# cule/multimot_track

Measured on AMD Instinct MI355X. Metric: KITTI RGB-D frames/sec (ego+object poses) at 1/2/4/8 GPUs; CPU ref fps, higher is better.
Workload: dtype u8

## Files before the change

multimot_track_amd/csrc/mmt_bowmap.hip:

```cpp

#include <algorithm>
#include <climits>
#include <cmath>
#include <cstring>
#include <functional>

#include "mmt_internal.h"
#include "mmt_map.h"
#include "mmt_mat4.h"
#include "mmt_pnp.h"

namespace mmt {

namespace {
constexpr int TH_LOW = 50, HISTO_LENGTH = 30;

void three_max(const std::vector<int>* histo, int& ind1, int& ind2, int& ind3) {
  int max1 = 0, max2 = 0, max3 = 0;
  for (int i = 0; i < HISTO_LENGTH; i++) {
    const int s = (int)histo[i].size();
    if (s > max1) {
      max3 = max2; max2 = max1; max1 = s;
      ind3 = ind2; ind2 = ind1; ind1 = i;
    } else if (s > max2) {
// ... 816 lines not shown
        const float errX1 = u1 - kp1.x, errY1 = v1 - kp1.y;
        if ((errX1 * errX1 + errY1 * errY1) > 5.991 * sigmaSquare1) continue;
      } else {
        const float u1 = cam_.fx * x1 * invz1 + cam_.cx;
        const float u1_r = u1 - cam_.bf * invz1;
        const float v1 = cam_.fy * y1 * invz1 + cam_.cy;
        const float errX1 = u1 - kp1.x, errY1 = v1 - kp1.y, errX1_r = u1_r - kp1_ur;
        if ((errX1 * errX1 + errY1 * errY1 + errX1_r * errX1_r) > 7.8 * sigmaSquare1) continue;
      }
      const float sc2 = cam_.scale[kp2.octave], sigmaSquare2 = sc2 * sc2;
      const float x2 = row_dot(T2, 0), y2 = row_dot(T2, 1);
      const float invz2 = (float)(1.0 / z2);
      if (!bStereo2) {
        const float u2 = cam_.fx * x2 * invz2 + cam_.cx, v2 = cam_.fy * y2 * invz2 + cam_.cy;
        const float errX2 = u2 - kp2.x, errY2 = v2 - kp2.y;
        if ((errX2 * errX2 + errY2 * errY2) > 5.991 * sigmaSquare2) continue;
      } else {
        const float u2 = cam_.fx * x2 * invz2 + cam_.cx;
        const float u2_r = u2 - cam_.bf * invz2;
        const float v2 = cam_.fy * y2 * invz2 + cam_.cy;
        const float errX2 = u2 - kp2.x, errY2 = v2 - kp2.y, errX2_r = u2_r - kp2_ur;
        if ((errX2 * errX2 + errY2 * errY2 + errX2_r * errX2_r) > 7.8 * sigmaSquare2) continue;
      }
      const float n1v[3] = {x3D[0] - kfs_[kf].Ow[0], x3D[1] - kfs_[kf].Ow[1], x3D[2] - kfs_[kf].Ow[2]};
      const float n2v[3] = {x3D[0] - kfs_[k2].Ow[0], x3D[1] - kfs_[k2].Ow[1], x3D[2] - kfs_[k2].Ow[2]};
      const float dist1 = norm3(n1v), dist2 = norm3(n2v);
      if (dist1 == 0 || dist2 == 0) continue;
      const float ratioDist = dist2 / dist1;
      const float ratioOctave = cam_.scale[kp1.octave] / cam_.scale[kp2.octave];
      if (ratioDist * ratioFactor < ratioOctave || ratioDist > ratioOctave * ratioFactor) continue;
      const int hnew = new_point_kf(x3D, kf);
      add_observation(hnew, kf, idx1);
      add_observation(hnew, k2, idx2);
      kfs_[kf].mps[idx1] = hnew;
      kfs_[k2].mps[idx2] = hnew;
      compute_distinctive(hnew);
      update_normal_depth(hnew);
      recent_.push_back(hnew);
      bstats_.n_triangulated++;
    }
  }
}

}
```

multimot_track_amd/csrc/mmt_localmap.hip:

```cpp

#include <hip/hip_runtime.h>

#include <algorithm>
#include <climits>
#include <cmath>
#include <cstring>
#include <map>
#include <set>

#include "mmt_map.h"
#include "mmt_mat4.h"

namespace mmt {

void MapEngine::grow_dev(uint8_t*& d, uint8_t*& h, size_t& cap, size_t need) {
  if (need <= cap && d) return;
  const size_t c = std::max(need + (need >> 1), (size_t)1 << 16);
  if (d) {
    MMT_HIP(hipStreamSynchronize(lm_s_));
    dallocs_.erase(std::find(dallocs_.begin(), dallocs_.end(), (void*)d));
    (void)hipFree(d);
    hallocs_.erase(std::find(hallocs_.begin(), hallocs_.end(), (void*)h));
    (void)hipHostFree(h);
  }
// ... 32 lines not shown
  memcpy(K.Tcw, T, 64);
  cam_centre(T, K.Ow);
  mat4_eye(K.Twc);
  for (int r = 0; r < 3; r++) {
    for (int c = 0; c < 3; c++) K.Twc[4 * r + c] = T[4 * c + r];
    K.Twc[4 * r + 3] = K.Ow[r];
  }
}

void MapEngine::erase_observation(int h, int kf) {
  MPoint& p = mp(h);
  auto it = std::lower_bound(p.obs.begin(), p.obs.end(), std::make_pair(kf, INT_MIN));
  if (it == p.obs.end() || it->first != kf) return;
  if (kfs_[kf].uR[it->second] >= 0)
    p.nObs -= 2;
  else
    p.nObs--;
  p.obs.erase(it);
  if (p.refKF == kf) p.refKF = p.obs.empty() ? -1 : p.obs.front().first;
  if (p.nObs <= 2) set_bad(h);
}

void MapEngine::replace(int h, int by) {
  if (h == by) return;
  MPoint& p = mp(h);
  const std::vector<std::pair<int, int>> obs = p.obs;
  p.obs.clear();
  mark_bad(h);
  const int nvisible = p.visible, nfound = p.found;
  p.replaced = by;
  mark_dirty(h);
  for (const auto& kv : obs) {
    if (mp(by).obs_index(kv.first) < 0) {
      kfs_[kv.first].mps[kv.second] = by;
      add_observation(by, kv.first, kv.second);
    } else {
      kfs_[kv.first].mps[kv.second] = -1;
    }
  }
  MPoint& q = mp(by);
  q.found += nfound;
  q.visible += nvisible;
  compute_distinctive(by);
}

void MapEngine::erase_connection(int kf, int other) {
  if (kfs_[kf].conn.erase(other)) update_best_covisibles(kf);
}

void MapEngine::kf_set_bad(int kf) {
  KFrame& K = kfs_[kf];
  if (K.id == 0) return;
  for (const auto& kv : std::map<int, int>(K.conn)) erase_connection(kv.first, kf);
  for (size_t i = 0; i < K.mps.size(); i++)
    if (K.mps[i] >= 0) erase_observation(K.mps[i], kf);
  K.conn.clear();
  K.ordered.clear();
  std::set<int> cand;
  cand.insert(K.parent);
  while (!K.children.empty()) {
    bool bContinue = false;
    int mx = -1, pC = -1, pP = -1;
    for (int ch : K.children) {
      if (kfs_[ch].bad) continue;
      for (int c : kfs_[ch].ordered)
        for (int q : cand)
          if (c == q) {
            auto it = kfs_[ch].conn.find(c);
            const int wgt = it == kfs_[ch].conn.end() ? 0 : it->second;
            if (wgt > mx) {
              pC = ch;
              pP = c;
              mx = wgt;
              bContinue = true;
            }
          }
    }
    if (!bContinue) break;
    kfs_[pC].parent = pP;
    kfs_[pP].children.insert(pC);
    mstats_.n_reparent++;
    cand.insert(pC);
    K.children.erase(pC);
  }
  if (K.parent >= 0) {
    for (int ch : K.children) {
      kfs_[ch].parent = K.parent;
      kfs_[K.parent].children.insert(ch);
      mstats_.n_reparent++;
    }
    kfs_[K.parent].children.erase(kf);
  }
  K.bad = true;
  kfdb_erase(kf);
}

void MapEngine::fuse_launch(const std::vector<int>& kft_kf, const std::vector<FuseQuery>& q,
                            int2* res) {
  const int nq = (int)q.size();
  if (nq == 0) return;
  const double t0 = prof_on_ ? now_us() : 0;
  double tq = t0;
  gpu_flush_pool(lm_s_);
  blk_time(10, tq);
  const size_t tb = al16(sizeof(FuseKF) * kft_kf.size());
  grow_dev(d_fup_, h_fup_, fup_cap_, tb + sizeof(FuseQuery) * (size_t)nq);
  {
    uint8_t* dres = (uint8_t*)d_fres_;
    uint8_t* hres = (uint8_t*)h_fres_;
    grow_dev(dres, hres, fres_cap_, sizeof(int2) * (size_t)nq);
    d_fres_ = (int2*)dres;
    h_fres_ = (int2*)hres;
  }
  FuseKF* tab = (FuseKF*)h_fup_;
  for (size_t t = 0; t < kft_kf.size(); t++) {
    const KFrame& K = kfs_[kft_kf[t]];
    tab[t] = K.dev;
    memcpy(tab[t].Tcw, K.Tcw, 64);
    memcpy(tab[t].Ow, K.Ow, 12);
  }
  memcpy(h_fup_ + tb, q.data(), sizeof(FuseQuery) * (size_t)nq);
  MMT_HIP(hipMemcpyAsync(d_fup_, h_fup_, tb + sizeof(FuseQuery) * (size_t)nq,
                         hipMemcpyHostToDevice, lm_s_));
  FuseCam c;
  memset(&c, 0, sizeof(c));
  c.fx = cam_.fx; c.fy = cam_.fy; c.cx = cam_.cx; c.cy = cam_.cy; c.bf = cam_.bf;
// ... 4 lines not shown
  c.logScale = cam_.logScale;
  c.th = 3.f;
  c.nlevels = cam_.nlevels;
  for (int l = 0; l < cam_.nlevels && l < kMaxLevels; l++) {
    c.scale[l] = cam_.scale[l];
    c.invSigma2[l] = cam_.invSigma2[l];
  }
  launch_fuse_cand((const FuseKF*)d_fup_, (const FuseQuery*)(d_fup_ + tb), nq, d_pool_,
                   d_pool_desc_, c, d_fres_, lm_s_);
  MMT_HIP(hipMemcpyAsync(h_fres_, d_fres_, sizeof(int2) * (size_t)nq, hipMemcpyDeviceToHost,
                         lm_s_));
  blk_time(11, tq);
  MMT_HIP(hipStreamSynchronize(lm_s_));
  blk_time(12, tq);
  memcpy(res, h_fres_, sizeof(int2) * (size_t)nq);
  mstats_.fuse_launches++;
  mstats_.fuse_queries += nq;
  if (prof_on_) mstats_.fuse_us += now_us() - t0;
}

void MapEngine::fuse_apply(int kf, int h, int bestIdx, int bestDist) {
  if (bestDist > 50) return;
  KFrame& K = kfs_[kf];
  const int pin = K.mps[bestIdx];
  if (pin >= 0) {
    if (!mp(pin).bad) {
      if (mp(pin).nObs > mp(h).nObs)
        replace(h, pin);
      else
        replace(pin, h);
    }
  } else {
    add_observation(h, kf, bestIdx);
    K.mps[bestIdx] = h;
  }
  mstats_.n_fused++;
}

void MapEngine::fuse_sequence(const std::vector<int>& kfl, const std::vector<int>& pts) {
  const int nk = (int)kfl.size(), np = (int)pts.size();
  if (nk == 0 || np == 0) return;
  std::vector<int> qidx((size_t)nk * np, -1);
  std::vector<FuseQuery> q;
  std::vector<int> ver;
  for (int t = 0; t < nk; t++)
    for (int i = 0; i < np; i++) {
      if (t == 0 && i + 8 < np) prefetch_point(pts[i + 8]);
      const int h = pts[i];
      if (h < 0 || mp(h).bad || mp(h).obs_index(kfl[t]) >= 0) continue;
      qidx[(size_t)t * np + i] = (int)q.size();
      q.push_back(FuseQuery{t, h});
      ver.push_back(mp(h).desc_ver);
    }
  std::vector<int2> res(q.size());
  double tb = prof_on_ ? now_us() : 0;
  fuse_launch(kfl, q, res.data());
  tb = prof_on_ ? now_us() : 0;
  for (int t = 0; t < nk; t++) {
    const int kf = kfl[t];
    for (int i = 0; i < np; i++) {
      const int h = pts[i];
      if (h < 0) continue;
      const MPoint& p = mp(h);
      if (p.bad || p.obs_index(kf) >= 0) continue;
      const int qi = qidx[(size_t)t * np + i];
      if (qi < 0) continue;
      if (ver[qi] != p.desc_ver) {
// ... 135 lines not shown
  for (int v = 0; v < nK; v++) vIdx[verts[v]] = -1;
  BAHostProblem P;
  P.n_kf = nK;
  P.n_pt = nP;
  P.n_edge = nE;
  P.Tcw = Tv.data();
  P.fixed = fixed.data();
  P.Xw = Xv.data();
  P.e_pt = e_pt.data();
  P.e_kf = e_kf.data();
  P.e_obs = e_obs.data();
  P.e_s = e_s.data();
  P.fx = cam_.fx; P.fy = cam_.fy; P.cx = cam_.cx; P.cy = cam_.cy; P.bf = cam_.bf;
  std::vector<float> Tout(16 * (size_t)nK), Xout(3 * (size_t)nP);
  std::vector<uint8_t> er(std::max(nE, 1));
  int st[5];
  double tb = prof_on_ ? now_us() : 0;
  if (prof_on_) mstats_.blk_us[8] += tb - t0;
  ba_.run(P, lm_s_, Tout.data(), Xout.data(), er.data(), st);
  if (prof_on_) mstats_.basolve_us += now_us() - tb;
  tb = prof_on_ ? now_us() : 0;
  mstats_.n_ba++;
  mstats_.ba_trials += st[2] + st[3];
  mstats_.ba_edges += nE;
  mstats_.ba_kfs += nK;
  mstats_.ba_pts += nP;
  mstats_.ba_max_opt = std::max<long>(mstats_.ba_max_opt, nO);
  for (int pass = 0; pass < 2; pass++)
    for (int i = 0; i < nE; i++) {
      const bool stereo = !(e_obs[3 * (size_t)i + 2] < 0);
      if (stereo != (pass == 1) || !er[i]) continue;
      const int h = lpts[e_pt[i]], k = e_kfid[i];
      const int idx = mp(h).obs_index(k);
      if (idx >= 0) kfs_[k].mps[idx] = -1;
      erase_observation(h, k);
      mstats_.n_ba_erased++;
    }
  for (size_t v = 0; v < local.size(); v++) set_pose(local[v], &Tout[16 * v]);
  for (int j = 0; j < nP; j++) {
    MPoint& p = mp(lpts[j]);
    memcpy(p.pos, &Xout[3 * (size_t)j], 12);
    mark_dirty(lpts[j]);
    update_normal_depth(lpts[j]);
  }
  blk_time(9, tb);
  if (prof_on_) mstats_.ba_us += now_us() - t0;
}

void MapEngine::keyframe_culling(int kf) {
  const std::vector<int> local = kfs_[kf].ordered;
  for (int k : local) {
    KFrame& K = kfs_[k];
    if (K.id == 0) continue;
    const int thObs = 3;
    int nRedundant = 0, nMPs = 0;
    for (size_t i = 0; i < K.mps.size(); i++) {
      const int h = K.mps[i];
      if (h < 0) continue;
      const MPoint& p = mp(h);
      if (p.bad) continue;
      if (K.depth[i] > cam_.thDepth || K.depth[i] < 0) continue;
      nMPs++;
      if (p.nObs > thObs) {
        const int scaleLevel = K.keys[i].octave;
        int nObs = 0;
        for (const auto& kv : p.obs) {
          if (kv.first == k) continue;
// ... 38 lines not shown
```

multimot_track_amd/csrc/mmt_map.h:

```cpp
#pragma once
#include <hip/hip_runtime.h>

#include <cstdint>
#include <functional>
#include <map>
#include <set>
#include <unordered_map>
#include <utility>
#include <memory>
#include <vector>

#include "mmt_ba.h"
#include "mmt_bow.h"
#include "mmt_internal.h"
#include "mmt_match.h"
#include "mmt_track.h"

namespace mmt {

struct MapCamH {
  int W = 0, H = 0;
  float fx = 0, fy = 0, cx = 0, cy = 0, invfx = 0, invfy = 0, bf = 0;
  float thDepth = 0;
  int maxFrames = 0;
// ... 150 lines not shown
    const double n = now_us();
    mstats_.blk_us[k] += n - t;
    t = n;
  }
  void prefetch_point(int h) const {
#ifndef MMT_NO_PREFETCH
    if (h >= 0 && h < kTemp && (size_t)h < pts_.size()) __builtin_prefetch(&pts_[h]);
#else
    (void)h;
#endif
  }
  void set_cull_ratio(double r) { cull_ratio_ = r; }
  void dump(int32_t* sizes, const mmt_map_dump_arrays* out) const;
  void set_vocabulary(Vocabulary* v);
  const BowStatsH& bow_stats() const { return bstats_; }

 private:
  std::function<void()> overlap_;
  std::vector<int> kf_count_, kf_touched_;
  std::vector<int> lp_buf_;
  std::vector<uint64_t> lp_seen_;
  bool spec_on_ = true, spec_valid_ = false;
  bool overlap_c3_ = true;
  long spec_frame_ = -1, spec_stamp_ = 0, spec_hits_ = 0, spec_tries_ = 0;
  std::vector<int> spec_mps_, spec_cnt_, spec_touched_, spec_kfs_, spec_pts_;
  std::vector<long> spec_mark_;
  uint8_t* h_early_ = nullptr;
  hipEvent_t ev_early_ = nullptr;
  void speculate_local_map(const MapFrameH& L, int n);
  bool commit_local_map(MapFrameH& C);
  void spec_discard();
  template <class Marked, class Mark>
  void expand_local_kfs(std::vector<int>& kfl, Marked marked, Mark mark);
  void collect_local_points(const std::vector<int>& kfl, std::vector<int>& out);
  struct DistCache {
    std::vector<uint64_t> ids;
    std::vector<uint16_t> d;
  };
  std::unordered_map<int, DistCache> dcache_;
  void run_overlap() {
    if (!overlap_) return;
    std::function<void()> fn = std::move(overlap_);
    overlap_ = nullptr;
    fn();
  }
  static constexpr int kTemp = 1 << 29;
  MPoint& mp(int h) { return h >= kTemp ? temps_[h - kTemp] : pts_[h]; }
  bool track_with_motion_model(MapFrameH& C, const GridFrame& G, float* Tcw, MapFrameH& L,
                               float* Tlast, const float* vel, MapStatsH& st);
  bool track_reference_subst(MapFrameH& C, const GridFrame& G, float* Tcw, const MapFrameH& L,
                             const float* Tlast);
  bool relocalization_subst(MapFrameH& C, const GridFrame& G, float* Tcw, const float* Tlast,
                            const float* vel);
  bool track_local_map(MapFrameH& C, const GridFrame& G, float* Tcw);
  int discard_outliers(MapFrameH& C, int nmatches, int* nmatchesMap);
  void update_last_frame(MapFrameH& L, float* Tlast);
  void update_local_keyframes(MapFrameH& C);
  void update_local_points();
  void search_local_points(MapFrameH& C, const GridFrame& G, const float* Tcw);
  bool need_new_keyframe(const MapFrameH& C);
  void create_new_keyframe(MapFrameH& C, const float* Tcw);
  int new_keyframe(const MapFrameH& C, const float* Tcw);
  int new_point_kf(const float* pos, int kf);
  void add_observation(int h, int kf, int idx);
  void set_bad(int h);
  void compute_distinctive(int h);
  void update_normal_depth(int h);
// ... 100 lines not shown
  uint8_t* d_last_ = nullptr;
  uint8_t* h_last_ = nullptr;
  CandSet c2_{};
  uint8_t* d_out_ = nullptr;
  uint8_t* h_out_ = nullptr;
  int* d_match_ = nullptr;
  int* d_nm_ = nullptr;
  int* h_match_ = nullptr;
  int* h_nm_ = nullptr;
  float* d_edges_ = nullptr;
  float* h_edges_ = nullptr;
  PoseOptDesc* d_pod_ = nullptr;
  PoseOptDesc* h_pod_ = nullptr;
  float* d_pose_ = nullptr;
  uint8_t* d_outl_ = nullptr;
  int* d_ninl_ = nullptr;
  double* d_esc_ = nullptr;
  int* d_fsc_ = nullptr;
  float* h_pose_ = nullptr;
  uint8_t* h_outl_ = nullptr;
  int* h_ninl_ = nullptr;
  LocalPointDev* d_pool_ = nullptr;
  uint8_t* d_pool_desc_ = nullptr;
  int pool_cap_ = 0;
  PoolUpdate* d_up_ = nullptr;
  PoolUpdate* h_up_ = nullptr;
  int up_cap_ = 0;
  uint8_t* d_sel_ = nullptr;
  uint8_t* h_sel_ = nullptr;
  uint8_t* d_inview_ = nullptr;
  uint8_t* h_inview_ = nullptr;
  CandSet c3_{};
  int local_cap_ = 0;
  GridFrame G_{};
  MappingStats mstats_;
  double cull_ratio_ = 0.9;
  hipStream_t lm_s_ = nullptr;
  std::vector<uint8_t*> kf_blocks_;
  size_t kf_rec_bytes_ = 0;
  static constexpr int kKFBlock = 64;
  uint8_t* d_fup_ = nullptr;
  uint8_t* h_fup_ = nullptr;
  size_t fup_cap_ = 0;
  int2* d_fres_ = nullptr;
  int2* h_fres_ = nullptr;
  size_t fres_cap_ = 0;
  BARunner ba_;
  std::vector<int> ba_vidx_;
  void grow_dev(uint8_t*& d, uint8_t*& h, size_t& cap, size_t need);
};

template <typename T>
inline T* MapEngine::dev(size_t n) {
  T* p = nullptr;
  MMT_HIP(hipMalloc((void**)&p, std::max<size_t>(n, 1) * sizeof(T)));
  dallocs_.push_back(p);
  return p;
}

template <typename T>
inline T* MapEngine::pinned(size_t n) {
  T* p = nullptr;
  MMT_HIP(hipHostMalloc((void**)&p, std::max<size_t>(n, 1) * sizeof(T), hipHostMallocDefault));
  hallocs_.push_back(p);
  return p;
}
// ... 3 lines not shown
```

multimot_track_amd/csrc/mmt_map.hip:

```cpp

#include <hip/hip_runtime.h>

#include <algorithm>
#include <climits>
#include <cstdio>
#include <cstdlib>
#include <cmath>
#include <cstring>

#include "mmt_map.h"
#include "mmt_mat4.h"

namespace mmt {

#define MAP_PROF(k, stmt)                       \
  do {                                          \
    const double _t0 = prof_on_ ? now_us() : 0; \
    stmt;                                       \
    if (prof_on_) prof_[k] += now_us() - _t0;   \
  } while (0)

MapEngine::~MapEngine() {
  if (prof_on_ && prof_n_ > 0) {
    static const char* names[12] = {"C2 search", "D1 (motion model)", "local map update",
                                    "C3 search", "D1 (local map)", "keyframe + mapping",
                                    "other", "total", "UpdateLastFrame", "C2 pack",
                                    "C3 pack", "D1 pack"};
    fprintf(stderr, "[mmt map profile] %ld frames, host wall us per frame:", prof_n_);
    for (int k = 0; k < 12; k++) fprintf(stderr, " %s %.1f%s", names[k], prof_[k] / prof_n_,
                                         k < 11 ? "," : "\n");
    if (mstats_.n_lm > 0) {
      const double n = (double)mstats_.n_lm;
      fprintf(stderr, "[mmt localmapping profile] %ld keyframes, host wall us per keyframe: "
              "ProcessNewKeyFrame+MapPointCulling %.1f, CreateNewMapPoints + SearchInNeighbors %.1f "
              "(CreateNewMapPoints %.1f, Fuse launches "
              "%.1f), LocalBundleAdjustment %.1f (solve %.1f), KeyFrameCulling %.1f, final sync "
              "%.1f, LocalMapping total %.1f; CreateNewKeyFrame with all of it %.1f\n", mstats_.n_lm,
              mstats_.pnk_us / n,
              mstats_.sin_us / n, mstats_.cnmp_us / n, mstats_.fuse_us / n, mstats_.ba_us / n,
              mstats_.basolve_us / n, mstats_.cull_us / n, mstats_.lmsync_us / n,
              mstats_.lm_us / n, mstats_.kfnew_us / n);
      static const char* bn[MappingStats::kBlk] = {
          "new keyframe + store", "new points", "SIN targets", "SIN fuse 1", "SIN candidates",
          "SIN fuse 2", "SIN point updates", "SIN connections", "BA graph", "BA apply",
          "Fuse pool flush", "Fuse enqueue", "Fuse wait", "Fuse apply (+ relaunches)",
          "ComputeDistinctiveDescriptors (inside the others)", "PNK ComputeBoW",
          "PNK observations", "PNK UpdateConnections"};
      fprintf(stderr, "[mmt localmapping profile] per keyframe, us:");
      for (int k = 0; k < MappingStats::kBlk; k++)
        fprintf(stderr, " %s %.1f%s", bn[k], mstats_.blk_us[k] / n,
                k + 1 < MappingStats::kBlk ? "," : "\n");
    }
    fprintf(stderr, "[mmt map profile] per frame: %.1f local keyframes, %.1f local points, "
            "%.1f C3 edges; %zu map points allocated, %d keyframes at the end; local map "
            "speculated %ld times, taken %ld\n",
            prof_cnt_[0] / prof_n_, prof_cnt_[1] / prof_n_, prof_cnt_[2] / prof_n_, pts_.size(),
            n_keyframes(), spec_tries_, spec_hits_);
  }
  if (s_) (void)hipStreamSynchronize(s_);
  if (lm_s_) {
    (void)hipStreamSynchronize(lm_s_);
    (void)hipStreamDestroy(lm_s_);
  }
  if (ev_early_) (void)hipEventDestroy(ev_early_);
  for (void* p : dallocs_) (void)hipFree(p);
  for (void* p : hallocs_) (void)hipHostFree(p);
}

static size_t last_bytes(int n) { return (size_t)n * (sizeof(mmt_kp) + 12 + 32 + 2); }

static_assert(sizeof(PoseOptDesc) <= kDescBytes, "PoseOptDesc outgrew its slot");
static size_t align16(size_t x) { return (x + 15) & ~(size_t)15; }

struct SelLayout {
  size_t ids, skip, taken, bX, bHas, total;
  SelLayout(int m, int n) {
    ids = kDescBytes;
    skip = ids + 4 * (size_t)m;
    taken = skip + m;
    bX = align16(taken + n);
    bHas = bX + 12 * (size_t)n;
    total = bHas + n;
  }
};

size_t MapEngine::out_bytes(int n) const { return kOutHdr + 4 * (size_t)kcap_ + n; }

void MapEngine::setup(const MapCamH& cam, int kcap) {
  cam_ = cam;
  kcap_ = kcap;
  d_last_ = dev<uint8_t>(kDescBytes + last_bytes(kcap));
  h_last_ = pinned<uint8_t>(kDescBytes + last_bytes(kcap));
  c2_ = CandSet{dev<uint32_t>((size_t)kcap * kCandK), dev<int>((size_t)kcap * kCandK),
                dev<int>(kcap), dev<PointWin>(kcap), dev<int>(kcap)};
  d_out_ = dev<uint8_t>(kOutHdr + 5 * (size_t)kcap);
  h_out_ = pinned<uint8_t>(kOutHdr + 5 * (size_t)kcap);
  d_nm_ = (int*)d_out_;
  d_ninl_ = (int*)(d_out_ + 4);
  d_pose_ = (float*)(d_out_ + 16);
  d_match_ = (int*)(d_out_ + kOutHdr);
  d_outl_ = d_out_ + kOutHdr + 4 * (size_t)kcap;
  h_nm_ = (int*)h_out_;
  h_ninl_ = (int*)(h_out_ + 4);
  h_pose_ = (float*)(h_out_ + 16);
  h_match_ = (int*)(h_out_ + kOutHdr);
  h_outl_ = h_out_ + kOutHdr + 4 * (size_t)kcap;
  d_edges_ = dev<float>(7 * (size_t)kcap);
  h_edges_ = pinned<float>(7 * (size_t)kcap);
  d_esc_ = dev<double>(3 * (size_t)kcap);
  d_fsc_ = dev<int>(kcap);
  prof_on_ = getenv("MMT_MAP_PROFILE") != nullptr;
  if (const char* e = getenv("MMT_LOCALMAP_SPEC")) spec_on_ = atoi(e) != 0;
  if (const char* e = getenv("MMT_OVERLAP_C3")) overlap_c3_ = atoi(e) != 0;
  h_early_ = pinned<uint8_t>(kOutHdr + 4 * (size_t)kcap);
  MMT_HIP(hipEventCreateWithFlags(&ev_early_, hipEventDisableTiming));
  int prio_lo = 0, prio_hi = 0;
  MMT_HIP(hipDeviceGetStreamPriorityRange(&prio_lo, &prio_hi));
  const char* lmp = getenv("MMT_LM_PRIO");
  const int lm_prio = lmp && strcmp(lmp, "high") == 0 ? prio_hi : 0;
  MMT_HIP(hipStreamCreateWithPriority(&lm_s_, hipStreamNonBlocking, lm_prio));
  kf_rec_bytes_ = align16(sizeof(mmt_kp) * (size_t)kcap) + 32 * (size_t)kcap +
                  align16(4 * (size_t)kcap) + align16(4 * (size_t)(kGridCells + 1)) +
                  align16(4 * (size_t)kcap);
  frameNextId_ = 0;
  mbVO_ = false;
  matchesInliers_ = 0;
  lastRelocFrameId_ = 0;
  reset();
}

void MapEngine::grow_local(int m) {
  if (m <= local_cap_ && d_sel_) return;
  const int cap = std::max(m + 4096, 2 * local_cap_);
  void* old[] = {d_sel_, h_sel_, d_inview_, h_inview_, c3_.key, c3_.idx, c3_.n, c3_.win,
                 c3_.choice};
  if (s_) MMT_HIP(hipStreamSynchronize(s_));
  for (int i = 0; i < 9; i++) {
    if (!old[i]) continue;
    auto it = std::find(i == 1 || i == 3 ? hallocs_.begin() : dallocs_.begin(),
                        i == 1 || i == 3 ? hallocs_.end() : dallocs_.end(), old[i]);
    if (i == 1 || i == 3) {
      (void)hipHostFree(old[i]);
      hallocs_.erase(it);
    } else {
      (void)hipFree(old[i]);
      dallocs_.erase(it);
    }
  }
  const size_t sel_cap = SelLayout(cap, kcap_).total + 16;
  d_sel_ = dev<uint8_t>(sel_cap);
  h_sel_ = pinned<uint8_t>(sel_cap);
  d_inview_ = dev<uint8_t>(cap);
  h_inview_ = pinned<uint8_t>(cap);
  c3_ = CandSet{dev<uint32_t>((size_t)cap * kCandK), dev<int>((size_t)cap * kCandK), dev<int>(cap),
                dev<PointWin>(cap), dev<int>(cap)};
  local_cap_ = cap;
}

void MapEngine::reset() {
  pts_.clear();
  hot_.clear();
  dcache_.clear();
  spec_discard();
  temps_.clear();
  kfs_.clear();
  state_ = 0;
  frameNextId_ = 0;
  kfNextId_ = 0;
  lastKFFrameId_ = 0;
  refKF_ = -1;
  localKFs_.clear();
  localPts_.clear();
  recent_.clear();
  dirty_.clear();
  hasTlr_ = false;
  snapKF_ = -1;
  n_good_ = 0;
  for (auto& l : invfile_) l.clear();
}

int MapEngine::n_keyframes() const {
  int n = 0;
  for (const KFrame& k : kfs_) n += !k.bad;
  return n;
}

void MapEngine::prepare(MapFrameH& F) const {
  F.mps.assign(F.n, -1);
  F.outlier.assign(F.n, 0);
  F.refKF = -1;
  F.hasBow = false;
  F.bow.word.clear();
  F.bow.value.clear();
  F.fv = FeatVecH();
}

void MapEngine::mark_dirty(int h) {
  if (h >= kTemp) return;
  MPoint& p = pts_[h];
  if (!p.dirty) {
    p.dirty = true;
    dirty_.push_back(h);
  }
}

int MapEngine::new_point_kf(const float* pos, int kf) {
  MPoint p;
  memcpy(p.pos, pos, 12);
  p.firstKFid = kfs_[kf].id;
  p.refKF = kf;
  pts_.push_back(p);
  hot_.push_back(PtHot());
  n_good_++;
  const int h = (int)pts_.size() - 1;
  mark_dirty(h);
  return h;
}

void MapEngine::add_observation(int h, int kf, int idx) {
  MPoint& p = mp(h);
  if (p.obs_index(kf) >= 0) return;
  auto it = std::lower_bound(p.obs.begin(), p.obs.end(), std::make_pair(kf, INT_MIN));
  p.obs.insert(it, {kf, idx});
  if (kfs_[kf].uR[idx] >= 0)
    p.nObs += 2;
  else
    p.nObs++;
}

void MapEngine::mark_bad(int h) {
  MPoint& p = mp(h);
  if (!p.bad && h < kTemp) n_good_--;
  p.bad = true;
  if (h < kTemp) hot_[h].bad = 1;
  if (!dcache_.empty()) dcache_.erase(h);
}

void MapEngine::set_bad(int h) {
  MPoint& p = mp(h);
  mark_bad(h);
  const std::vector<std::pair<int, int>> o = p.obs;
  p.obs.clear();
  for (const auto& kv : o) kfs_[kv.first].mps[kv.second] = -1;
  mark_dirty(h);
}

void MapEngine::compute_distinctive(int h) {
  MPoint& p = mp(h);
  if (p.bad || p.obs.empty()) return;
  struct Timer {
    MapEngine* m;
    double t;
    ~Timer() {
      if (m) m->mstats_.blk_us[14] += now_us() - t;
    }
  } timer{prof_on_ ? this : nullptr, prof_on_ ? now_us() : 0};
  constexpr int kStack = 32;
  const uint8_t* Ds[kStack];
  std::vector<const uint8_t*> Dh;
  std::vector<uint64_t> ids;
  int N = 0;
  for (const auto& kv : p.obs)
    if (!kfs_[kv.first].bad) {
      const uint8_t* d = kfs_[kv.first].desc.data() + 32 * (size_t)kv.second;
      if (N < kStack) Ds[N] = d;
      if (N == kStack) Dh.assign(Ds, Ds + kStack);
      if (N >= kStack) Dh.push_back(d);
      ids.push_back(((uint64_t)(uint32_t)kv.first << 32) | (uint32_t)kv.second);
      N++;
    }
  if (N == 0) return;
  const uint8_t* const* Dv = N <= kStack ? Ds : Dh.data();
  int dist_s[kStack * kStack], v_s[kStack];
  std::vector<int> dist_h, v_h;
  if (N > kStack) {
    dist_h.assign((size_t)N * N, 0);
// ... 58 lines not shown
    const float* Ow = kfs_[kv.first].Ow;
    const float ni[3] = {p.pos[0] - Ow[0], p.pos[1] - Ow[1], p.pos[2] - Ow[2]};
    const double inv = 1.0 / (double)norm3(ni);
    for (int k = 0; k < 3; k++) normal[k] = normal[k] + (float)((double)ni[k] * inv);
    n++;
  }
  const KFrame& R = kfs_[p.refKF];
  const float PC[3] = {p.pos[0] - R.Ow[0], p.pos[1] - R.Ow[1], p.pos[2] - R.Ow[2]};
  const float dist = norm3(PC);
  const int level = R.keys[p.obs_index(p.refKF)].octave;
  p.maxDist = dist * cam_.scale[level];
  p.minDist = p.maxDist / cam_.scale[cam_.nlevels - 1];
  for (int k = 0; k < 3; k++) p.normal[k] = (float)((double)normal[k] * (1.0 / n));
  mark_dirty(h);
}

int MapEngine::new_keyframe(const MapFrameH& C, const float* Tcw) {
  kfs_.emplace_back();
  KFrame& k = kfs_.back();
  k.id = kfNextId_++;
  k.frameId = C.id;
  memcpy(k.Tcw, Tcw, 64);
  cam_centre(Tcw, k.Ow);
  mat4_eye(k.Twc);
  for (int r = 0; r < 3; r++) {
    for (int c = 0; c < 3; c++) k.Twc[4 * r + c] = Tcw[4 * c + r];
    k.Twc[4 * r + 3] = k.Ow[r];
  }
  k.keys.assign(C.kps, C.kps + C.n);
  k.uR.assign(C.uR, C.uR + C.n);
  k.depth.assign(C.depth, C.depth + C.n);
  k.desc.assign(C.desc, C.desc + 32 * (size_t)C.n);
  k.mps = C.mps;
  return (int)kfs_.size() - 1;
}

void MapEngine::update_best_covisibles(int kf) {
  KFrame& K = kfs_[kf];
  std::vector<std::pair<int, int>> v;
  for (const auto& kv : K.conn) v.push_back({kv.second, kv.first});
  std::sort(v.begin(), v.end());
  K.ordered.clear();
  for (auto it = v.rbegin(); it != v.rend(); ++it) K.ordered.push_back(it->second);
}

void MapEngine::add_connection(int kf, int other, int w) {
  KFrame& K = kfs_[kf];
  auto it = K.conn.find(other);
  if (it == K.conn.end())
    K.conn[other] = w;
  else if (it->second != w)
    it->second = w;
  else
    return;
  update_best_covisibles(kf);
}

void MapEngine::update_connections(int kf) {
  std::map<int, int> counter;
  for (int h : kfs_[kf].mps) {
    if (h < 0) continue;
    const MPoint& p = mp(h);
    if (p.bad) continue;
    for (const auto& kv : p.obs)
      if (kv.first != kf) counter[kv.first]++;
  }
  if (counter.empty()) return;
  int nmax = 0, kmax = -1;
  std::vector<std::pair<int, int>> v;
  for (const auto& kv : counter) {
    if (kv.second > nmax) {
      nmax = kv.second;
      kmax = kv.first;
    }
    if (kv.second >= 15) {
      v.push_back({kv.second, kv.first});
      add_connection(kv.first, kf, kv.second);
    }
  }
  if (v.empty()) {
    v.push_back({nmax, kmax});
    add_connection(kmax, kf, nmax);
  }
  std::sort(v.begin(), v.end());
  KFrame& K = kfs_[kf];
  K.conn = counter;
  K.ordered.clear();
  for (auto it = v.rbegin(); it != v.rend(); ++it) K.ordered.push_back(it->second);
  if (K.firstConnection && K.id != 0) {
    K.parent = K.ordered.front();
    kfs_[K.parent].children.insert(kf);
    K.firstConnection = false;
  }
}

int MapEngine::tracked_map_points(int kf, int minObs) {
  int n = 0;
  for (int h : kfs_[kf].mps) {
    if (h < 0) continue;
    const MPoint& p = mp(h);
    if (p.bad) continue;
    if (minObs > 0) {
      if (p.nObs >= minObs) n++;
    } else {
      n++;
    }
  }
  return n;
}

void MapEngine::process_new_keyframe(int kf) {
  double tb = prof_on_ ? now_us() : 0;
  if (voc_) kf_bow_launch(kf);
  blk_time(15, tb);
  const std::vector<int> mps = kfs_[kf].mps;
  for (size_t i = 0; i < mps.size(); i++) {
    const int h = mps[i];
    if (h < 0 || mp(h).bad) continue;
    if (mp(h).obs_index(kf) < 0) {
// ... 239 lines not shown
  out->kf_mps_start[kfs_.size()] = (int32_t)sl;
  long b = 0;
  for (size_t j = 0; j < pts_.size(); j++) {
    const MPoint& p = pts_[j];
    float* f = out->pt_f + 5 * j;
    memcpy(f, p.pos, 12);
    f[3] = p.minDist; f[4] = p.maxDist;
    int32_t* pi = out->pt_i + 5 * j;
    pi[0] = p.bad; pi[1] = p.nObs; pi[2] = p.refKF; pi[3] = p.firstKFid; pi[4] = p.replaced;
    out->obs_start[j] = (int32_t)b;
    for (const auto& ob : p.obs) {
      const KFrame& K = kfs_[ob.first];
      int32_t* oi = out->obs_i + 3 * b;
      float* of = out->obs_f + 4 * b;
      oi[0] = ob.first; oi[1] = ob.second; oi[2] = K.keys[ob.second].octave;
      of[0] = K.keys[ob.second].x; of[1] = K.keys[ob.second].y;
      of[2] = K.depth[ob.second]; of[3] = K.uR[ob.second];
      b++;
    }
  }
  out->obs_start[pts_.size()] = (int32_t)b;
}

void MapEngine::initialize(MapFrameH& C, const float* Tcw) {
  const int kf = new_keyframe(C, Tcw);
  kf_store_add(kf);
  for (int i = 0; i < C.n; i++) {
    const float z = C.depth[i];
    if (z > 0) {
      float x3D[3];
      unproject(cam_, Tcw, C.kps[i].x, C.kps[i].y, z, x3D);
      const int h = new_point_kf(x3D, kf);
      add_observation(h, kf, i);
      kfs_[kf].mps[i] = h;
      compute_distinctive(h);
      update_normal_depth(h);
      C.mps[i] = h;
    }
  }
  process_new_keyframe(kf);
  map_point_culling(kf);
  local_mapping(kf);
  lastKFFrameId_ = C.id;
  localKFs_.assign(1, kf);
  localPts_.clear();
  for (size_t h = 0; h < pts_.size(); h++)
    if (!pts_[h].bad) localPts_.push_back((int)h);
  refKF_ = kf;
  C.refKF = kf;
  state_ = 1;
}

void MapEngine::frame_done(const MapFrameH& C, const float* Tcw) {
  const int snap = snapKF_;
  snapKF_ = -1;
  if (C.refKF < 0) return;
  mat4_mul(Tcw, C.refKF == snap ? snapTwc_ : kfs_[C.refKF].Twc, Tlr_);
  hasTlr_ = true;
}

void MapEngine::update_last_frame(MapFrameH& L, float* Tlast) {
  if (L.refKF >= 0 && hasTlr_) mat4_mul(Tlr_, kfs_[L.refKF].Tcw, Tlast);
  if (lastKFFrameId_ == L.id) return;
  auto make = [&](int i) {
    if (L.mps[i] < 0 || mp(L.mps[i]).nObs < 1) {
      MPoint p;
      unproject(cam_, Tlast, L.kps[i].x, L.kps[i].y, L.depth[i], p.pos);
      memcpy(p.desc, L.desc + 32 * (size_t)i, 32);
      temps_.push_back(p);
      L.mps[i] = kTemp + (int)temps_.size() - 1;
    }
  };
  temps_.reserve(L.n);
  far_.clear();
  int nclose = 0;
  for (int i = 0; i < L.n; i++) {
    const float z = L.depth[i];
    if (!(z > 0)) continue;
    if (z > cam_.thDepth) {
      far_.push_back({z, i});
// ... 139 lines not shown
    const MPoint& p = mp(C.mps[i]);
    if (!p.bad) {
      for (const auto& kv : p.obs)
        if (kf_count_[kv.first]++ == 0) kf_touched_.push_back(kv.first);
    } else {
      C.mps[i] = -1;
    }
  }
  if (kf_touched_.empty()) return;
  std::sort(kf_touched_.begin(), kf_touched_.end());
  int mx = 0, kmax = -1;
  localKFs_.clear();
  for (const int id : kf_touched_) {
    const int cnt = kf_count_[id];
    kf_count_[id] = 0;
    KFrame& K = kfs_[id];
    if (K.bad) continue;
    if (cnt > mx) {
      mx = cnt;
      kmax = id;
    }
    localKFs_.push_back(id);
    K.trackRef = curId_;
  }
  expand_local_kfs(
      localKFs_, [&](int id) { return kfs_[id].trackRef == curId_; },
      [&](int id) { kfs_[id].trackRef = curId_; });
  if (kmax >= 0) {
    refKF_ = kmax;
    C.refKF = kmax;
  }
}

void MapEngine::update_local_points() { collect_local_points(localKFs_, localPts_); }

void MapEngine::collect_local_points(const std::vector<int>& kfl, std::vector<int>& out) {
  out.clear();
  std::vector<int>& buf = lp_buf_;
  const size_t words = (hot_.size() + 63) / 64;
  if (lp_seen_.size() < words) lp_seen_.resize(words, 0);
  for (int kf : kfl) {
    const std::vector<int>& mps = kfs_[kf].mps;
    buf.resize(mps.size());
    size_t n = 0;
    for (int h : mps) {
      buf[n] = h;
      n += (unsigned)h < (unsigned)kTemp;
    }
    for (size_t i = 0; i < n; i++) {
      const int h = buf[i];
      uint64_t& wd = lp_seen_[(size_t)h >> 6];
      const uint64_t bit = 1ull << (h & 63);
      if (wd & bit) continue;
      if (!hot_[h].bad) {
        out.push_back(h);
        wd |= bit;
      }
    }
  }
  for (int h : out) lp_seen_[(size_t)h >> 6] &= ~(1ull << (h & 63));
}

void MapEngine::speculate_local_map(const MapFrameH& L, int n) {
  spec_discard();
  const int* match = (const int*)(h_early_ + kOutHdr);
  if (spec_cnt_.size() < kfs_.size()) spec_cnt_.resize(kfs_.size(), 0);
  if (spec_mark_.size() < kfs_.size()) spec_mark_.resize(kfs_.size(), 0);
  spec_mps_.assign(n, -1);
  spec_touched_.clear();
  for (int i = 0; i < n; i++) {
    if (match[i] < 0) continue;
    const int h = L.mps[match[i]];
    spec_mps_[i] = h;
    if (h < 0) continue;
    const MPoint& p = mp(h);
    if (p.bad) continue;
    for (const auto& kv : p.obs)
      if (spec_cnt_[kv.first]++ == 0) spec_touched_.push_back(kv.first);
  }
  std::sort(spec_touched_.begin(), spec_touched_.end());
  const long stamp = ++spec_stamp_;
  spec_kfs_.clear();
  for (const int id : spec_touched_)
    if (!kfs_[id].bad) {
      spec_kfs_.push_back(id);
      spec_mark_[id] = stamp;
    }
  spec_frame_ = curId_;
  if (spec_kfs_.empty()) return;
  expand_local_kfs(
      spec_kfs_, [&](int id) { return spec_mark_[id] == stamp; },
      [&](int id) { spec_mark_[id] = stamp; });
  collect_local_points(spec_kfs_, spec_pts_);
  spec_valid_ = true;
  spec_tries_++;
}

void MapEngine::spec_discard() {
  for (const int id : spec_touched_) spec_cnt_[id] = 0;
  spec_touched_.clear();
  spec_valid_ = false;
}

bool MapEngine::commit_local_map(MapFrameH& C) {
  if (!spec_valid_ || spec_frame_ != curId_ || (int)spec_mps_.size() != C.n) {
    spec_discard();
    return false;
  }
  bool ok = true;
  for (int i = 0; i < C.n && ok; i++) {
    const int h = C.mps[i], s0 = spec_mps_[i];
    if (h >= 0 && h != s0) {
      ok = false;
    } else if (s0 >= 0 && h < 0) {
      const MPoint& p = mp(s0);
      if (!p.bad)
        for (const auto& kv : p.obs) spec_cnt_[kv.first]--;
    }
  }
  for (size_t q = 0; q < spec_touched_.size() && ok; q++) {
    const int id = spec_touched_[q];
    ok = kfs_[id].bad || spec_cnt_[id] > 0;
  }
  if (!ok) {
    spec_discard();
    return false;
  }
  for (int i = 0; i < C.n; i++)
    if (C.mps[i] >= 0 && mp(C.mps[i]).bad) C.mps[i] = -1;
  int mx = 0, kmax = -1;
  for (const int id : spec_touched_) {
    const int cnt = spec_cnt_[id];
    spec_cnt_[id] = 0;
    if (kfs_[id].bad) continue;
    if (cnt > mx) {
      mx = cnt;
      kmax = id;
    }
  }
  spec_touched_.clear();
  spec_valid_ = false;
  for (const int id : spec_kfs_) kfs_[id].trackRef = curId_;
  localKFs_.swap(spec_kfs_);
  localPts_.swap(spec_pts_);
  if (kmax >= 0) {
    refKF_ = kmax;
    C.refKF = kmax;
  }
  spec_hits_++;
  return true;
}

void MapEngine::search_local_points(MapFrameH& C, const GridFrame& G, const float* Tcw) {
  const double t_pack = prof_on_ ? now_us() : 0;
  for (int i = 0; i < C.n; i++) {
    if (C.mps[i] < 0) continue;
    const int h = C.mps[i];
    MPoint& p = mp(h);
    if (p.bad) {
      C.mps[i] = -1;
    } else {
      p.visible++;
      p.lastSeen = curId_;
      if (h < kTemp) hot_[h].lastSeen = (int)curId_;
      p.trackInView = false;
    }
  }
  const int m = (int)localPts_.size();
  grow_local(m);
  gpu_flush_pool();
  const SelLayout sl(m, C.n);
  int* ids = (int*)(h_sel_ + sl.ids);
  uint8_t* skip = h_sel_ + sl.skip;
  uint8_t* taken = h_sel_ + sl.taken;
  for (int j = 0; j < m; j++) {
    const int h = localPts_[j];
    const PtHot& q = hot_[h];
    ids[j] = h;
    skip[j] = q.lastSeen == (int)curId_ || q.bad;
  }
  float* bX = (float*)(h_sel_ + sl.bX);
  uint8_t* bHas = h_sel_ + sl.bHas;
  int nbase = 0;
  for (int i = 0; i < C.n; i++) {
    const int h = C.mps[i];
    taken[i] = 0;
    bHas[i] = h >= 0;
    if (h >= 0) {
      const MPoint& p = mp(h);
      taken[i] = p.nObs > 0;
      memcpy(bX + 3 * (size_t)i, p.pos, 12);
      nbase++;
    }
  }
  if (prof_on_) prof_[10] += now_us() - t_pack;
  pose_desc_fill(h_sel_, d_sel_, Tcw);
  MMT_HIP(hipMemcpyAsync(d_sel_, h_sel_, sl.total, hipMemcpyHostToDevice, s_));
  const float th = curId_ < lastRelocFrameId_ + 2 ? 5.f : 3.f;
  LocalSel sel{(const int*)(d_sel_ + sl.ids), d_sel_ + sl.skip, d_inview_};
  MapEdgeArgs e = edge_args(G);
  e.pool = d_pool_;
  e.ids = (const int*)(d_sel_ + sl.ids);
  e.has_base = d_sel_ + sl.bHas;
  e.base_X = (const float*)(d_sel_ + sl.bX);
  launch_search_local(G, Tcw, d_pool_, d_pool_desc_, m, th, d_sel_ + sl.taken, nullptr, c3_,
                      d_match_, d_nm_, s_, &sel, &e);
  launch_pose_opt(d_pod_, 1, std::min(C.n, nbase + m), s_);
  MMT_HIP(hipMemcpyAsync(h_out_, d_out_, out_bytes(C.n), hipMemcpyDeviceToHost, s_));
  if (m > 0) MMT_HIP(hipMemcpyAsync(h_inview_, d_inview_, (size_t)m, hipMemcpyDeviceToHost, s_));
  run_overlap();
  MMT_HIP(hipStreamSynchronize(s_));
  for (int j = 0; j < m; j++)
    if (!skip[j] && h_inview_[j]) mp(localPts_[j]).visible++;
  for (int i = 0; i < C.n; i++)
    if (h_match_[i] >= 0) C.mps[i] = localPts_[h_match_[i]];
}

bool MapEngine::track_local_map(MapFrameH& C, const GridFrame& G, float* Tcw) {
  MAP_PROF(2, if (!commit_local_map(C)) {
    update_local_keyframes(C);
    update_local_points();
  });
  if (prof_on_) {
    prof_cnt_[0] += localKFs_.size();
    prof_cnt_[1] += localPts_.size();
  }
  MAP_PROF(3, search_local_points(C, G, Tcw));
  MAP_PROF(4, apply_pose_opt(C, Tcw));
  matchesInliers_ = 0;
  for (int i = 0; i < C.n; i++) {
    if (C.mps[i] < 0 || C.outlier[i]) continue;
    MPoint& p = mp(C.mps[i]);
    p.found++;
    if (p.nObs > 0) matchesInliers_++;
  }
// ... 44 lines not shown
      key.push_back(b);
      v.push_back(i);
    }
  if (!v.empty()) {
    const int nv = (int)v.size();
    std::vector<int> pos(nv);
    for (int k = 0; k < nv; k++) pos[k] = k;
    tmp.resize(nv);
    for (int pass = 0; pass < 3; pass++) {
      uint32_t cnt[2049];
      memset(cnt, 0, sizeof(cnt));
      const int sh = 11 * pass;
      for (int k = 0; k < nv; k++) cnt[((key[pos[k]] >> sh) & 0x7FF) + 1]++;
      for (int b = 0; b < 2048; b++) cnt[b + 1] += cnt[b];
      for (int k = 0; k < nv; k++) tmp[cnt[(key[pos[k]] >> sh) & 0x7FF]++] = pos[k];
      pos.swap(tmp);
    }
    int nPoints = 0;
    for (int j = 0; j < nv; j++) {
      const int i = v[pos[j]];
      const float depth_i = C.depth[i];
      bool create = false;
      if (C.mps[i] < 0) {
        create = true;
      } else if (mp(C.mps[i]).nObs < 1) {
        create = true;
        C.mps[i] = -1;
      }
      if (create) {
        float x3D[3];
        unproject(cam_, Tcw, C.kps[i].x, C.kps[i].y, C.depth[i], x3D);
        const int h = new_point_kf(x3D, kf);
        add_observation(h, kf, i);
        kfs_[kf].mps[i] = h;
        compute_distinctive(h);
        update_normal_depth(h);
        C.mps[i] = h;
      }
      nPoints++;
      if (depth_i > cam_.thDepth && nPoints > 200) break;
    }
  }
  blk_time(1, tb);
  snapKF_ = kf;
  memcpy(snapTwc_, kfs_[kf].Twc, sizeof(snapTwc_));
  const double tp = prof_on_ ? now_us() : 0;
  process_new_keyframe(kf);
  map_point_culling(kf);
  if (prof_on_) mstats_.pnk_us += now_us() - tp;
  local_mapping(kf);
  if (voc_ && kfs_[kf].id != 0 && !kfs_[kf].bad) kfdb_add(kf);
  lastKFFrameId_ = C.id;
}

int MapEngine::track(MapFrameH& C, const GridFrame& G, float* Tcw, MapFrameH& L, float* Tlast,
                     float* vel, bool& has_vel, bool& bSecondFrame, MapStatsH& st,
                     hipStream_t s) {
  s_ = s;
  curId_ = C.id;
  const double t_track = prof_on_ ? now_us() : 0;
  bool bOK;
  if (has_vel)
    mat4_mul(vel, Tlast, Tcw);
  else
    memcpy(Tcw, Tlast, 64);
  if (state_ == 1) {
    for (int i = 0; i < L.n; i++)
// ... 79 lines not shown
```

Measured before the change: 713.6.

## Cache local map point lists keyed by keyframe set and structure epoch

Adds a small LRU cache of local point lists, keyed by the local keyframe list and invalidated by a structure epoch counter. Every map-point/keyframe association edit, bad-marking or covisibility update bumps that counter. On a hit the walk over keyframe observations is skipped. The point id array also moves to its own device buffer and is uploaded only when the list generation changes, which shrinks the per-frame host-to-device copy. The risk is stale lists if some mutation path misses the epoch bump; a verify mode (2) compares the cached list against a fresh walk.

```diff
diff --git a/multimot_track_amd/csrc/mmt_bowmap.hip b/multimot_track_amd/csrc/mmt_bowmap.hip
--- a/multimot_track_amd/csrc/mmt_bowmap.hip
+++ b/multimot_track_amd/csrc/mmt_bowmap.hip
@@ -872,8 +872,8 @@
       const int hnew = new_point_kf(x3D, kf);
       add_observation(hnew, kf, idx1);
       add_observation(hnew, k2, idx2);
-      kfs_[kf].mps[idx1] = hnew;
-      kfs_[k2].mps[idx2] = hnew;
+      kf_set_mp(kf, idx1, hnew);
+      kf_set_mp(k2, idx2, hnew);
       compute_distinctive(hnew);
       update_normal_depth(hnew);
       recent_.push_back(hnew);
diff --git a/multimot_track_amd/csrc/mmt_localmap.hip b/multimot_track_amd/csrc/mmt_localmap.hip
--- a/multimot_track_amd/csrc/mmt_localmap.hip
+++ b/multimot_track_amd/csrc/mmt_localmap.hip
@@ -88,10 +88,10 @@
   mark_dirty(h);
   for (const auto& kv : obs) {
     if (mp(by).obs_index(kv.first) < 0) {
-      kfs_[kv.first].mps[kv.second] = by;
+      kf_set_mp(kv.first, kv.second, by);
       add_observation(by, kv.first, kv.second);
     } else {
-      kfs_[kv.first].mps[kv.second] = -1;
+      kf_set_mp(kv.first, kv.second, -1);
     }
   }
   MPoint& q = mp(by);
@@ -148,6 +148,7 @@
     kfs_[K.parent].children.erase(kf);
   }
   K.bad = true;
+  struct_epoch_++;
   kfdb_erase(kf);
 }
 
@@ -218,7 +219,7 @@
     }
   } else {
     add_observation(h, kf, bestIdx);
-    K.mps[bestIdx] = h;
+    kf_set_mp(kf, bestIdx, h);
   }
   mstats_.n_fused++;
 }
@@ -420,7 +421,7 @@
       if (stereo != (pass == 1) || !er[i]) continue;
       const int h = lpts[e_pt[i]], k = e_kfid[i];
       const int idx = mp(h).obs_index(k);
-      if (idx >= 0) kfs_[k].mps[idx] = -1;
+      if (idx >= 0) kf_set_mp(k, idx, -1);
       erase_observation(h, k);
       mstats_.n_ba_erased++;
     }
diff --git a/multimot_track_amd/csrc/mmt_map.h b/multimot_track_amd/csrc/mmt_map.h
--- a/multimot_track_amd/csrc/mmt_map.h
+++ b/multimot_track_amd/csrc/mmt_map.h
@@ -206,7 +206,26 @@
   void spec_discard();
   template <class Marked, class Mark>
   void expand_local_kfs(std::vector<int>& kfl, Marked marked, Mark mark);
-  void collect_local_points(const std::vector<int>& kfl, std::vector<int>& out);
+  void collect_local_points(const std::vector<int>& kfl, std::vector<int>& out, long& gen);
+  void walk_local_points(const std::vector<int>& kfl, std::vector<int>& out);
+  long struct_epoch_ = 0;
+  void kf_set_mp(int kf, int idx, int h) {
+    kfs_[kf].mps[idx] = h;
+    struct_epoch_++;
+  }
+  int lpc_mode_ = 1, lpc_ways_ = 4;
+  struct LpcEntry {
+    std::vector<int> kfs, pts;
+    long gen = 0, used = 0;
+    bool valid = false;
+  };
+  static constexpr int kLpcMaxWays = 8;
+  LpcEntry lpc_[kLpcMaxWays];
+  std::vector<int> lpc_check_;
+  long lpc_epoch_ = -1, lpc_tick_ = 0, lpc_hits_ = 0, lpc_rebuilds_ = 0, lpc_new_epoch_ = 0;
+  long ids_uploads_ = 0;
+  long list_gen_ = 0;
+  long local_gen_ = 0, spec_gen_ = 0;
   struct DistCache {
     std::vector<uint64_t> ids;
     std::vector<uint16_t> d;
@@ -373,6 +392,9 @@
   uint8_t* h_inview_ = nullptr;
   CandSet c3_{};
   int local_cap_ = 0;
+  int* d_ids_ = nullptr;
+  int* h_ids_ = nullptr;
+  long ids_gen_ = -1;
   GridFrame G_{};
   MappingStats mstats_;
   double cull_ratio_ = 0.9;
diff --git a/multimot_track_amd/csrc/mmt_map.hip b/multimot_track_amd/csrc/mmt_map.hip
--- a/multimot_track_amd/csrc/mmt_map.hip
+++ b/multimot_track_amd/csrc/mmt_map.hip
@@ -53,9 +53,11 @@
     }
     fprintf(stderr, "[mmt map profile] per frame: %.1f local keyframes, %.1f local points, "
             "%.1f C3 edges; %zu map points allocated, %d keyframes at the end; local map "
-            "speculated %ld times, taken %ld\n",
+            "speculated %ld times, taken %ld; local point list cache (MMT_LOCALMAP_CACHE=%d) "
+            "hits %ld, rebuilds %ld (%ld of them after a structure edit, %ld ids uploads)\n",
             prof_cnt_[0] / prof_n_, prof_cnt_[1] / prof_n_, prof_cnt_[2] / prof_n_, pts_.size(),
-            n_keyframes(), spec_tries_, spec_hits_);
+            n_keyframes(), spec_tries_, spec_hits_, lpc_mode_, lpc_hits_, lpc_rebuilds_,
+            lpc_new_epoch_, ids_uploads_);
   }
   if (s_) (void)hipStreamSynchronize(s_);
   if (lm_s_) {
@@ -74,9 +76,9 @@
 
 struct SelLayout {
   size_t ids, skip, taken, bX, bHas, total;
-  SelLayout(int m, int n) {
+  SelLayout(int m, int n, bool ids_inline = true) {
     ids = kDescBytes;
-    skip = ids + 4 * (size_t)m;
+    skip = ids + (ids_inline ? 4 * (size_t)m : 0);
     taken = skip + m;
     bX = align16(taken + n);
     bHas = bX + 12 * (size_t)n;
@@ -112,6 +114,9 @@
   prof_on_ = getenv("MMT_MAP_PROFILE") != nullptr;
   if (const char* e = getenv("MMT_LOCALMAP_SPEC")) spec_on_ = atoi(e) != 0;
   if (const char* e = getenv("MMT_OVERLAP_C3")) overlap_c3_ = atoi(e) != 0;
+  if (const char* e = getenv("MMT_LOCALMAP_CACHE")) lpc_mode_ = std::min(2, std::max(0, atoi(e)));
+  if (const char* e = getenv("MMT_LOCALMAP_CACHE_WAYS"))
+    lpc_ways_ = std::min(kLpcMaxWays, std::max(1, atoi(e)));
   h_early_ = pinned<uint8_t>(kOutHdr + 4 * (size_t)kcap);
   MMT_HIP(hipEventCreateWithFlags(&ev_early_, hipEventDisableTiming));
   int prio_lo = 0, prio_hi = 0;
@@ -133,13 +138,14 @@
   if (m <= local_cap_ && d_sel_) return;
   const int cap = std::max(m + 4096, 2 * local_cap_);
   void* old[] = {d_sel_, h_sel_, d_inview_, h_inview_, c3_.key, c3_.idx, c3_.n, c3_.win,
-                 c3_.choice};
+                 c3_.choice, d_ids_, h_ids_};
   if (s_) MMT_HIP(hipStreamSynchronize(s_));
-  for (int i = 0; i < 9; i++) {
+  for (int i = 0; i < 11; i++) {
     if (!old[i]) continue;
-    auto it = std::find(i == 1 || i == 3 ? hallocs_.begin() : dallocs_.begin(),
-                        i == 1 || i == 3 ? hallocs_.end() : dallocs_.end(), old[i]);
-    if (i == 1 || i == 3) {
+    const bool host = i == 1 || i == 3 || i == 10;
+    auto it = std::find(host ? hallocs_.begin() : dallocs_.begin(),
+                        host ? hallocs_.end() : dallocs_.end(), old[i]);
+    if (host) {
       (void)hipHostFree(old[i]);
       hallocs_.erase(it);
     } else {
@@ -154,6 +160,9 @@
   h_inview_ = pinned<uint8_t>(cap);
   c3_ = CandSet{dev<uint32_t>((size_t)cap * kCandK), dev<int>((size_t)cap * kCandK), dev<int>(cap),
                 dev<PointWin>(cap), dev<int>(cap)};
+  d_ids_ = dev<int>(cap);
+  h_ids_ = pinned<int>(cap);
+  ids_gen_ = -1;
   local_cap_ = cap;
 }
 
@@ -171,6 +180,8 @@
   refKF_ = -1;
   localKFs_.clear();
   localPts_.clear();
+  local_gen_ = ++list_gen_;
+  struct_epoch_++;
   recent_.clear();
   dirty_.clear();
   hasTlr_ = false;
@@ -232,7 +243,10 @@
   MPoint& p = mp(h);
   if (!p.bad && h < kTemp) n_good_--;
   p.bad = true;
-  if (h < kTemp) hot_[h].bad = 1;
+  if (h < kTemp) {
+    hot_[h].bad = 1;
+    struct_epoch_++;
+  }
   if (!dcache_.empty()) dcache_.erase(h);
 }
 
@@ -241,7 +255,7 @@
   mark_bad(h);
   const std::vector<std::pair<int, int>> o = p.obs;
   p.obs.clear();
-  for (const auto& kv : o) kfs_[kv.first].mps[kv.second] = -1;
+  for (const auto& kv : o) kf_set_mp(kv.first, kv.second, -1);
   mark_dirty(h);
 }
 
@@ -366,6 +380,7 @@
   k.depth.assign(C.depth, C.depth + C.n);
   k.desc.assign(C.desc, C.desc + 32 * (size_t)C.n);
   k.mps = C.mps;
+  struct_epoch_++;
   return (int)kfs_.size() - 1;
 }
 
@@ -376,6 +391,7 @@
   std::sort(v.begin(), v.end());
   K.ordered.clear();
   for (auto it = v.rbegin(); it != v.rend(); ++it) K.ordered.push_back(it->second);
+  struct_epoch_++;
 }
 
 void MapEngine::add_connection(int kf, int other, int w) {
@@ -419,6 +435,7 @@
   std::sort(v.begin(), v.end());
   KFrame& K = kfs_[kf];
   K.conn = counter;
+  struct_epoch_++;
   K.ordered.clear();
   for (auto it = v.rbegin(); it != v.rend(); ++it) K.ordered.push_back(it->second);
   if (K.firstConnection && K.id != 0) {
@@ -724,7 +741,7 @@
       unproject(cam_, Tcw, C.kps[i].x, C.kps[i].y, z, x3D);
       const int h = new_point_kf(x3D, kf);
       add_observation(h, kf, i);
-      kfs_[kf].mps[i] = h;
+      kf_set_mp(kf, i, h);
       compute_distinctive(h);
       update_normal_depth(h);
       C.mps[i] = h;
@@ -734,10 +751,12 @@
   map_point_culling(kf);
   local_mapping(kf);
   lastKFFrameId_ = C.id;
+  struct_epoch_++;
   localKFs_.assign(1, kf);
   localPts_.clear();
   for (size_t h = 0; h < pts_.size(); h++)
     if (!pts_[h].bad) localPts_.push_back((int)h);
+  local_gen_ = ++list_gen_;
   refKF_ = kf;
   C.refKF = kf;
   state_ = 1;
@@ -943,9 +962,53 @@
   }
 }
 
-void MapEngine::update_local_points() { collect_local_points(localKFs_, localPts_); }
-
-void MapEngine::collect_local_points(const std::vector<int>& kfl, std::vector<int>& out) {
+void MapEngine::update_local_points() {
+  collect_local_points(localKFs_, localPts_, local_gen_);
+}
+
+void MapEngine::collect_local_points(const std::vector<int>& kfl, std::vector<int>& out,
+                                     long& gen) {
+  LpcEntry* hit = nullptr;
+  if (lpc_mode_ != 0 && lpc_epoch_ == struct_epoch_)
+    for (int w = 0; w < lpc_ways_ && !hit; w++)
+      if (lpc_[w].valid && lpc_[w].kfs == kfl) hit = &lpc_[w];
+  if (hit) {
+    if (gen != hit->gen) {
+      out = hit->pts;
+      gen = hit->gen;
+    }
+    hit->used = ++lpc_tick_;
+    lpc_hits_++;
+    if (lpc_mode_ == 2) {
+      walk_local_points(kfl, lpc_check_);
+      if (lpc_check_ != out)
+        throw DeviceError("local point list cache: the cached list differs from the walk's (" +
+                          std::to_string(out.size()) + " / " + std::to_string(lpc_check_.size()) +
+                          " points, frame " + std::to_string(curId_) + ")");
+    }
+    return;
+  }
+  walk_local_points(kfl, out);
+  gen = ++list_gen_;
+  lpc_rebuilds_++;
+  if (lpc_mode_ != 0) {
+    if (lpc_epoch_ != struct_epoch_) {
+      lpc_new_epoch_++;
+      for (LpcEntry& e : lpc_) e.valid = false;
+      lpc_epoch_ = struct_epoch_;
+    }
+    LpcEntry* v = &lpc_[0];
+    for (int w = 0; w < lpc_ways_ && v->valid; w++)
+      if (!lpc_[w].valid || lpc_[w].used < v->used) v = &lpc_[w];
+    v->kfs = kfl;
+    v->pts = out;
+    v->gen = gen;
+    v->used = ++lpc_tick_;
+    v->valid = true;
+  }
+}
+
+void MapEngine::walk_local_points(const std::vector<int>& kfl, std::vector<int>& out) {
   out.clear();
   std::vector<int>& buf = lp_buf_;
   const size_t words = (hot_.size() + 63) / 64;
@@ -1002,7 +1065,7 @@
   expand_local_kfs(
       spec_kfs_, [&](int id) { return spec_mark_[id] == stamp; },
       [&](int id) { spec_mark_[id] = stamp; });
-  collect_local_points(spec_kfs_, spec_pts_);
+  collect_local_points(spec_kfs_, spec_pts_, spec_gen_);
   spec_valid_ = true;
   spec_tries_++;
 }
@@ -1054,6 +1117,7 @@
   for (const int id : spec_kfs_) kfs_[id].trackRef = curId_;
   localKFs_.swap(spec_kfs_);
   localPts_.swap(spec_pts_);
+  std::swap(local_gen_, spec_gen_);
   if (kmax >= 0) {
     refKF_ = kmax;
     C.refKF = kmax;
@@ -1080,14 +1144,19 @@
   const int m = (int)localPts_.size();
   grow_local(m);
   gpu_flush_pool();
-  const SelLayout sl(m, C.n);
-  int* ids = (int*)(h_sel_ + sl.ids);
+  const bool ids_inline = lpc_mode_ == 0;
+  const SelLayout sl(m, C.n, ids_inline);
+  const bool ids_new = ids_inline || ids_gen_ != local_gen_;
+  int* ids = ids_inline ? (int*)(h_sel_ + sl.ids) : h_ids_;
+  const int* d_ids = ids_inline ? (const int*)(d_sel_ + sl.ids) : d_ids_;
   uint8_t* skip = h_sel_ + sl.skip;
   uint8_t* taken = h_sel_ + sl.taken;
+  if (ids_new) {
+    memcpy(ids, localPts_.data(), 4 * (size_t)m);
+    ids_uploads_++;
+  }
   for (int j = 0; j < m; j++) {
-    const int h = localPts_[j];
-    const PtHot& q = hot_[h];
-    ids[j] = h;
+    const PtHot& q = hot_[localPts_[j]];
     skip[j] = q.lastSeen == (int)curId_ || q.bad;
   }
   float* bX = (float*)(h_sel_ + sl.bX);
@@ -1107,11 +1176,15 @@
   if (prof_on_) prof_[10] += now_us() - t_pack;
   pose_desc_fill(h_sel_, d_sel_, Tcw);
   MMT_HIP(hipMemcpyAsync(d_sel_, h_sel_, sl.total, hipMemcpyHostToDevice, s_));
+  if (!ids_inline && ids_new) {
+    if (m > 0) MMT_HIP(hipMemcpyAsync(d_ids_, h_ids_, 4 * (size_t)m, hipMemcpyHostToDevice, s_));
+    ids_gen_ = local_gen_;
+  }
   const float th = curId_ < lastRelocFrameId_ + 2 ? 5.f : 3.f;
-  LocalSel sel{(const int*)(d_sel_ + sl.ids), d_sel_ + sl.skip, d_inview_};
+  LocalSel sel{d_ids, d_sel_ + sl.skip, d_inview_};
   MapEdgeArgs e = edge_args(G);
   e.pool = d_pool_;
-  e.ids = (const int*)(d_sel_ + sl.ids);
+  e.ids = d_ids;
   e.has_base = d_sel_ + sl.bHas;
   e.base_X = (const float*)(d_sel_ + sl.bX);
   launch_search_local(G, Tcw, d_pool_, d_pool_desc_, m, th, d_sel_ + sl.taken, nullptr, c3_,
@@ -1222,7 +1295,7 @@
         unproject(cam_, Tcw, C.kps[i].x, C.kps[i].y, C.depth[i], x3D);
         const int h = new_point_kf(x3D, kf);
         add_observation(h, kf, i);
-        kfs_[kf].mps[i] = h;
+        kf_set_mp(kf, i, h);
         compute_distinctive(h);
         update_normal_depth(h);
         C.mps[i] = h;
```

Result: faster. 754.2 (median of 6 runs) (+5.7%).
